# Anaesthesiaye/sound_event_detection_transformer

Measured on AMD Instinct MI355X. Metric: audio clips/sec training throughput (B=64, 10s@64-mel), higher is better.
Workload: dtype bf16; 1 GPU; URBAN-SED SEDT enc_layers=3 dec_at num_queries=10 B=64/GPU, 10 s @ 64-mel (B,1,500,64), full train step: fwd + Hungarian matching (device) + SetCriterion + bwd + clip 0.1 + AdamW, dropout 0.1; global_batch=64, parallelism=dp1

## Files before the change

include/sedt_hip.h:

```cpp
#ifndef SEDT_HIP_H
#define SEDT_HIP_H
#include <stddef.h>
#include <stdint.h>

#ifdef __cplusplus
extern "C" {
#endif

#define SEDT_F32 0
#define SEDT_BF16 1
#define SEDT_BF16X3 2

#define SEDT_ACT_NONE 0
#define SEDT_ACT_RELU 1
#define SEDT_ACT_SIGMOID 2

const char* sedt_last_error(void);
int sedt_version(void);

typedef struct SedtIgemm {
  int32_t M, N, K;
  const void* A;
  const void* B;
  int64_t lda, ldb;
  int32_t trans, conv, transposed;
  int32_t Hi, Wi, Ci, Ho, Wo;
  int32_t KH, KW, sh, sw, ph, pw, dh, dw;
  void* C;
  int64_t ldc;
  int32_t out_f32;
  const float* scale;
  const float* bias;
  const void* res;
  int64_t ldr;
  int32_t res_mod;
  const void* mask;
  int64_t ldm;
  int32_t act, act_post_res;
  float alpha;
  float drop_p;
  uint32_t seed;
  const uint32_t* seed_ptr;
  int32_t splitk;
  float* slab;
  int32_t tile_m, tile_n;
  float* colsum_out;
  uint8_t* bits_out;
  int64_t ldbits;
  int32_t mask_bits;
  int32_t f32ep;
  int32_t omap;
  int32_t o_Hi, o_Wi, o_sh, o_sw, o_h0, o_w0;
  int32_t btap_on;
  int32_t btap[8];
  void* split_out;
  int32_t awrap;
  int32_t pad2_;
  const void* bfrag;
} SedtIgemm;

int sedt_igemm(const SedtIgemm* args, int dtype, void* stream);
int sedt_sizeof(int which);
int sedt_igemm_group(const SedtIgemm* jobs, int njobs, int dtype, void* stream);
int sedt_wgrad_group(const SedtIgemm* jobs, int njobs, int dtype, void* stream);
int sedt_igemm_co(const SedtIgemm* main, const SedtIgemm* wjobs, int nw, int dtype, void* stream, int* taken);
int sedt_igemm_splitk(int M, int N, int K, int dtype);
int sedt_igemm_describe(const SedtIgemm* args, int dtype, int grouped, char* out, int cap);
int sedt_igemm_group_describe(const SedtIgemm* jobs, int njobs, int dtype, char* out, int cap);

int sedt_wgrad_reduce(const float* slab, int splitk, int R, int taps, int Ci, const float* rowscale,
                      float* out, void* stream);
int sedt_wgrad_reduce_bias(const float* slab, int splitk, int R, int taps, int Ci, const float* rowscale, float* out,
                           const float* colsum_slab, float* bias_out, void* stream);

typedef struct SedtPrefetch {
  const void* ptr[3];
  size_t bytes[3];
} SedtPrefetch;

typedef struct SedtSplitJob {
  const float* src;
  int64_t ld;
  void* dst;
  int32_t rows, cols, pattern;
  int32_t blk0;
} SedtSplitJob;
int sedt_split3(const SedtSplitJob* jobs, int njobs, void* stream);

#define SEDT_MAX_REDUCE_JOBS 40
typedef struct SedtReduceJob {
  const float* slab;
  const float* rowscale;
// ... 337 lines not shown
```

sound_event_detection_transformer_amd/csrc/igemm.hip:

```cpp
#include <stdlib.h>
#include "common.h"

namespace sedt {

template <typename T> struct Cfg;
template <> struct Cfg<float> {
  static constexpr int BK = 32, PITCH = 33, EPC = 4, KSTEP = 2, UK = 1;
};
template <> struct Cfg<bf16_t> {
  static constexpr int BK = 64, PITCH = 72, EPC = 8, KSTEP = 16, UK = 4;
};

struct GatherGeom {
  int Hi, Wi, Ci, Ho, Wo, KH, KW, sh, sw, ph, pw, dh, dw, transposed;
};

__device__ __forceinline__ long gather_pix(const GatherGeom& g, int n, int ho, int wo, int kh, int kw) {
  int hi, wi;
  if (!g.transposed) {
    hi = ho * g.sh - g.ph + kh * g.dh;
    wi = wo * g.sw - g.pw + kw * g.dw;
    if ((unsigned)hi >= (unsigned)g.Hi || (unsigned)wi >= (unsigned)g.Wi) return -1;
  } else {
    int th = ho + g.ph - kh * g.dh, tw = wo + g.pw - kw * g.dw;
// ... 369 lines not shown
#pragma unroll
        for (int j = 0; j < NI; ++j) b[j] = cB[j * 32 * PITCH + kk + kofs];
#pragma unroll
        for (int i = 0; i < MI; ++i)
#pragma unroll
          for (int j = 0; j < NI; ++j)
            acc[i][j] = __builtin_amdgcn_mfma_f32_32x32x2f32(a[i], b[j], acc[i][j], 0, 0, 0);
      }
    }
  };

  if (nkb > 0) {
    load_tiles(kb_begin, ra0, rb0);
    if (nkb > 1) load_tiles(kb_begin + 1, ra1, rb1);
    store_tiles(0, ra0, rb0);
    __syncthreads();
    auto body = [&](int it, uint4(&fa)[NRA], uint4(&fb)[NRB], const uint4(&na)[NRA], const uint4(&nb)[NRB]) {
      if (it + 2 < nkb) load_tiles(kb_begin + it + 2, fa, fb);
      compute(it & 1);
      if (it + 1 < nkb) store_tiles((it & 1) ^ 1, na, nb);
      __syncthreads();
    };
    for (int it = 0; it < nkb; it += 2) {
      body(it, ra0, rb0, ra1, rb1);
      if (it + 1 < nkb) body(it + 1, ra1, rb1, ra0, rb0);
    }
  }

  const bool slab = p.splitk > 1;
  const uint32_t seed = eff_seed(p.seed, p.seed_ptr);
  const uint32_t thresh = drop_threshold(p.drop_p);
  const float inv_keep = p.drop_p > 0.f ? 1.f / (1.f - p.drop_p) : 1.f;
  const T* resT = reinterpret_cast<const T*>(p.res);
  const T* maskT = p.mask_bits ? nullptr : reinterpret_cast<const T*>(p.mask);
  const uint8_t* maskB = p.mask_bits ? reinterpret_cast<const uint8_t*>(p.mask) : nullptr;
  auto epilogue_tile = [&](const f32x16& a, const int i, const int j) {
    const int col = n0 + wn + j * 32 + (lane & 31);
    const bool colok = col < p.N;
    float sc = 1.f, bi = 0.f;
    if (!slab && colok) {
      if (p.scale) sc = p.scale[col];
      if (p.bias) bi = p.bias[col];
    }
#pragma unroll
    for (int r = 0; r < 16; ++r) {
      const int row = m0 + wm + i * 32 + (r & 3) + 8 * (r >> 2) + 4 * (lane >> 5);
      if (p.bits_out && !slab) {
        const bool ok = row < p.M && colok;
        float v = 0.f;
        if (ok) {
          v = a[r] * sc + bi;
          if (!p.act_post_res) {
            if (p.act == SEDT_ACT_RELU) v = fmaxf(v, 0.f);
            else if (p.act == SEDT_ACT_SIGMOID) v = 1.f / (1.f + __expf(-v));
          }
          if (p.drop_p > 0.f) v = drop_keep(seed, (uint64_t)row * (uint64_t)p.N + col, thresh) ? v * inv_keep : 0.f;
          if (resT) {
            long rr = p.res_mod > 0 ? (row % p.res_mod) : row;
            v += (float)resT[rr * p.ldr + col];
          }
          if (p.act_post_res) {
            if (p.act == SEDT_ACT_RELU) v = fmaxf(v, 0.f);
            else if (p.act == SEDT_ACT_SIGMOID) v = 1.f / (1.f + __expf(-v));
          }
          if (maskT) v = ((float)maskT[(long)row * p.ldm + col] > 0.f) ? v : 0.f;
          if (maskB) v = ((maskB[(long)row * p.ldm + (col >> 3)] >> (col & 7)) & 1) ? v : 0.f;
          v *= p.alpha;
          if (p.out_f32) reinterpret_cast<float*>(p.C)[(long)row * p.ldc + col] = v;
          else { const T tv = (T)v; reinterpret_cast<T*>(p.C)[(long)row * p.ldc + col] = tv; v = (float)tv; }
        }
        const unsigned long long pos = __ballot(ok && v > 0.f);
        if (ok && (lane & 7) == 0) p.bits_out[(long)row * p.ldbits + (col >> 3)] = (uint8_t)(pos >> (lane & ~7));
        continue;
      }
      if (!(row < p.M && colok)) continue;
      float v = a[r];
      if (slab) {
        p.slab[((long)blockIdx.z * p.M + row) * p.N + col] = v;
        continue;
      }
      v = v * sc + bi;
      if (!p.act_post_res) {
        if (p.act == SEDT_ACT_RELU) v = fmaxf(v, 0.f);
        else if (p.act == SEDT_ACT_SIGMOID) v = 1.f / (1.f + __expf(-v));
      }
      if (p.drop_p > 0.f) v = drop_keep(seed, (uint64_t)row * (uint64_t)p.N + col, thresh) ? v * inv_keep : 0.f;
      if (resT) {
        long rr = p.res_mod > 0 ? (row % p.res_mod) : row;
        v += (float)resT[rr * p.ldr + col];
      }
      if (p.act_post_res) {
        if (p.act == SEDT_ACT_RELU) v = fmaxf(v, 0.f);
        else if (p.act == SEDT_ACT_SIGMOID) v = 1.f / (1.f + __expf(-v));
      }
      if (maskT) v = ((float)maskT[(long)row * p.ldm + col] > 0.f) ? v : 0.f;
      if (maskB) v = ((maskB[(long)row * p.ldm + (col >> 3)] >> (col & 7)) & 1) ? v : 0.f;
      v *= p.alpha;
      if (p.out_f32) reinterpret_cast<float*>(p.C)[(long)row * p.ldc + col] = v;
      else reinterpret_cast<T*>(p.C)[(long)row * p.ldc + col] = (T)v;
    }
  };
  epilogue_tile(acc[0][0], 0, 0);
  if constexpr (NI > 1) epilogue_tile(acc[0][1], 0, 1);
  if constexpr (MI > 1) epilogue_tile(acc[1][0], 1, 0);
  if constexpr (MI > 1 && NI > 1) epilogue_tile(acc[1][1], 1, 1);
}

template <typename T, int BM, int BN, bool TRANS, bool X3 = false, bool FAST = false>
static int launch_cfg(const SedtIgemm& p, int vecA, int vecB, hipStream_t st) {
  if constexpr (!FAST && sizeof(T) == 4) {
    if (vecA && vecB && p.M % BM == 0 && p.N % BN == 0 && p.K % (X3 ? X3BK : Cfg<T>::BK) == 0 && (!p.conv || p.trans || p.Ci % (X3 ? X3BK : Cfg<T>::BK) == 0))
      return launch_cfg<T, BM, BN, TRANS, X3, true>(p, vecA, vecB, st);
  }
  SEDT_DESCRIBE("igemm_kernel<%s, %d, %d, %s%s%s>", sizeof(T) == 4 ? "float" : "__bf16", BM, BN, TRANS ? "true" : "false", X3 ? ", true" : "",
                FAST ? (X3 ? ", true" : ", false, true") : "");
  constexpr size_t lds = X3 ? (size_t)(BM + BN) * X3P * sizeof(bf16_t) * 2 * 2 : (size_t)(BM + BN) * Cfg<T>::PITCH * sizeof(T) * 2;
  static bool attr_set = false;
  auto kern = igemm_kernel<T, BM, BN, TRANS, X3, FAST>;
  if (!attr_set) {
    hipError_t e = hipFuncSetAttribute(reinterpret_cast<const void*>(kern), hipFuncAttributeMaxDynamicSharedMemorySize,
                                       (int)lds);
    if (e != hipSuccess) {
// ... 20 lines not shown
    if (!p.trans) SEDT_REQUIRE(p.Ci % (X3 ? X3BK : Cfg<T>::BK) == 0, "igemm: conv needs Ci %% BK == 0 (Ci=%d, BK=%d)", p.Ci, X3 ? X3BK : Cfg<T>::BK);
  }
  if (!p.trans) {
    if (p.K % EPC != 0) { vecA = 0; vecB = 0; }
  }
  int bm = p.tile_m, bn = p.tile_n;
  if (bm == 0 || bn == 0) {
    bm = 64; bn = 64;
    static int gen_tile = [] { const char* e = dev_getenv("SEDT_GEN_TILE"); return e ? atoi(e) : 0; }();
    static int gen_min = [] { const char* e = dev_getenv("SEDT_GEN_TILE_MIN"); return e ? atoi(e) : 512; }();
    if (gen_tile && sizeof(T) == 4) {
      const int tm = gen_tile / 1000 >= 128 ? 128 : 64, tn = gen_tile % 1000 >= 128 ? 128 : 64;
      if (p.M % tm == 0 && p.N % tn == 0 && (long)(p.M / tm) * (p.N / tn) * (p.splitk > 1 ? p.splitk : 1) >= gen_min) { bm = tm; bn = tn; }
    }
  }
  if (p.splitk > 1) SEDT_REQUIRE(p.slab != nullptr, "igemm: splitk > 1 needs a slab");
#define SEDT_DISPATCH(BM_, BN_)                                                         \
  if (bm == BM_ && bn == BN_) {                                                         \
    return p.trans ? launch_cfg<T, BM_, BN_, true, X3>(p, vecA, vecB, st)               \
                   : launch_cfg<T, BM_, BN_, false, X3>(p, vecA, vecB, st);             \
  }
  SEDT_DISPATCH(128, 128)
  SEDT_DISPATCH(128, 64)
  SEDT_DISPATCH(64, 64)
#undef SEDT_DISPATCH
  set_error("igemm: unsupported tile %dx%d", bm, bn);
  return 1;
}

}

namespace sedt { int igemm_lds_try(const SedtIgemm& p, hipStream_t st); }

static bool use_lds_family() {
  static int v = -1;
  if (v < 0) {
    const char* e = sedt::dev_getenv("SEDT_IGEMM_LDS");
    v = (e && e[0] == '0') ? 0 : 1;
  }
  return v == 1;
}

extern "C" int sedt_igemm(const SedtIgemm* args, int dtype, void* stream) {
  using namespace sedt;
  SEDT_REQUIRE(args != nullptr, "igemm: null args");
  SEDT_REQUIRE(args->M > 0 && args->N > 0 && args->K > 0, "igemm: bad dims M=%d N=%d K=%d", args->M, args->N, args->K);
  SEDT_REQUIRE(args->A && args->B && (args->C || args->splitk > 1), "igemm: null operand");
  hipStream_t st = reinterpret_cast<hipStream_t>(stream);
  if (dtype != SEDT_BF16)
    SEDT_REQUIRE(!args->omap && !args->btap_on && !args->f32ep && !args->awrap, "igemm: omap / btap / f32ep / awrap are features of the bf16 LDS-DMA kernels");
  if (dtype == SEDT_F32) {
    SEDT_REQUIRE(args->colsum_out == nullptr, "igemm: colsum_out is a bf16-only feature");
    return launch_typed<float>(*args, st);
  }
  if (dtype == SEDT_BF16X3) {
    SEDT_REQUIRE(args->colsum_out == nullptr, "igemm: colsum_out is a bf16-only feature");
    return launch_typed<float, true>(*args, st);
  }
  if (dtype == SEDT_BF16) {
    if (use_lds_family()) {
      int r = igemm_lds_try(*args, st);
      if (r >= 0) return r;
    }
    SEDT_REQUIRE(args->colsum_out == nullptr, "igemm: colsum_out needs the bf16 LDS-DMA wgrad kernel (M,N,lda,ldb %% 8 == 0)");
    SEDT_REQUIRE(!args->omap && !args->btap_on && !args->f32ep && !args->awrap,
                 "igemm: omap / btap / f32ep / awrap problem outside the LDS-DMA envelope (M %d N %d K %d)", args->M, args->N, args->K);
    return launch_typed<bf16_t>(*args, st);
  }
  set_error("igemm: unsupported dtype %d", dtype);
  return 1;
}

namespace sedt {
thread_local Describe describe = {false, {0}};
bool wgrad4_ok(const SedtIgemm& p);
int wgrad_lds_envelope(const SedtIgemm& p, long* a_bytes, long* b_bytes);
}

extern "C" int sedt_igemm_describe(const SedtIgemm* args, int dtype, int grouped, char* out, int cap) {
  using namespace sedt;
  SEDT_REQUIRE(args && out && cap > 0, "igemm_describe: bad arguments");
  out[0] = 0;
  if (grouped && dtype == SEDT_BF16 && args->trans) {
    long a, b;
    if (wgrad_lds_envelope(*args, &a, &b) == 0) {
      snprintf(out, cap, "%s", wgrad4_ok(*args) ? "wgrad4_group_kernel" : "wgrad3_group_kernel");
      return 0;
    }
  }
  describe.on = true;
  describe.name[0] = 0;
  const int r = sedt_igemm(args, dtype, nullptr);
  describe.on = false;
  if (r == 0) snprintf(out, cap, "%s", describe.name);
  return r;
}

namespace sedt {
int wgrad3_group_try(const SedtIgemm* jobs, int njobs, hipStream_t st);
bool wgrad4_shape_ok(int M, int N);
int wgrad4_tile_m(int M, int N);
int igemm3_group_try(const SedtIgemm* jobs, int njobs, hipStream_t st);
}

extern "C" int sedt_igemm_group(const SedtIgemm* jobs, int njobs, int dtype, void* stream) {
  SEDT_REQUIRE(jobs && njobs >= 1, "igemm_group: bad arguments");
  if (dtype == SEDT_BF16 && njobs >= 2) {
    const int r = sedt::igemm3_group_try(jobs, njobs, reinterpret_cast<hipStream_t>(stream));
    if (r >= 0) return r;
  }
  for (int i = 0; i < njobs; ++i)
    if (int r = sedt_igemm(&jobs[i], dtype, stream)) return r;
  return 0;
}

extern "C" int sedt_igemm_group_describe(const SedtIgemm* jobs, int njobs, int dtype, char* out, int cap) {
  using namespace sedt;
  SEDT_REQUIRE(jobs && njobs >= 1 && out && cap > 0, "igemm_group_describe: bad arguments");
  out[0] = 0;
  if (dtype != SEDT_BF16 || njobs < 2) return 0;
  describe.on = true;
  describe.name[0] = 0;
  const int r = igemm3_group_try(jobs, njobs, nullptr);
  describe.on = false;
  if (r == 0) snprintf(out, cap, "%s", describe.name);
  return r > 0 ? r : 0;
}

extern "C" int sedt_wgrad_group(const SedtIgemm* jobs, int njobs, int dtype, void* stream) {
  SEDT_REQUIRE(jobs && njobs >= 1, "wgrad_group: bad arguments");
  if (dtype == SEDT_BF16) {
    const int r = sedt::wgrad3_group_try(jobs, njobs, reinterpret_cast<hipStream_t>(stream));
    if (r >= 0) return r;
  }
  for (int i = 0; i < njobs; ++i)
    if (int r = sedt_igemm(&jobs[i], dtype, stream)) return r;
  return 0;
}

#include "wgrad3_body.h"
namespace sedt {
int wgrad3_group_build(const SedtIgemm* jobs, int njobs, WgradGroup* g);
extern thread_local const WgradGroup* co_group;
extern thread_local bool co_taken;
}

extern "C" int sedt_igemm_co(const SedtIgemm* main, const SedtIgemm* wjobs, int nw, int dtype, void* stream, int* taken) {
  using namespace sedt;
  SEDT_REQUIRE(main && (nw == 0 || wjobs) && taken, "igemm_co: bad arguments");
  *taken = 0;
  if (nw == 0) return sedt_igemm(main, dtype, stream);
  static int on = -1;
  if (on < 0) {
    const char* e = sedt::dev_getenv("SEDT_COSCHEDULE");
    on = (e && e[0] == '0') ? 0 : 1;
  }
  WgradGroup g;
  bool grouped = on && dtype == SEDT_BF16 && main->trans == 0 && wgrad3_group_build(wjobs, nw, &g) == 0;
  co_taken = false;
  co_group = grouped ? &g : nullptr;
  const int r = sedt_igemm(main, dtype, stream);
  co_group = nullptr;
  *taken = co_taken ? 1 : 0;
  return r;
}

extern "C" int sedt_igemm_splitk(int M, int N, int K, int dtype) {
  static int target_env = -2;
  if (target_env == -2) {
    const char* e = sedt::dev_getenv("SEDT_SPLITK_TARGET");
    target_env = e ? atoi(e) : -1;
  }
  const int target = target_env > 0 ? target_env : (dtype == SEDT_BF16 ? 384 : 768);
  int bk = dtype == SEDT_BF16 ? 64 : 32;
  long tiles = (long)((M + 63) / 64) * ((N + 63) / 64);
  int nkb = (K + bk - 1) / bk;
  int tgt = target;
  if (dtype == SEDT_BF16 && sedt::wgrad4_shape_ok(M, N)) {
    static int wide_env = -2;
    if (wide_env == -2) {
      const char* e = sedt::dev_getenv("SEDT_SPLITK_TARGET_WIDE");
      wide_env = e ? atoi(e) : -1;
    }
// ... 28 lines not shown
```

sound_event_detection_transformer_amd/csrc/igemm3.hip:

```cpp
#include <stdlib.h>
#include <type_traits>
#include "wgrad3_body.h"

namespace sedt {

__device__ __forceinline__ int uniform_i32(int v) { return __builtin_amdgcn_readfirstlane(v); }
typedef __attribute__((ext_vector_type(4))) unsigned u32x4;

__device__ __attribute__((used)) unsigned char g_code_tail_pad[64 * 1024];

#ifdef SEDT_DEV
__device__ unsigned long long g_phase_ts[5 * 4096];
__device__ int g_ts_filter[3];
#define SEDT_TS_INIT() \
  const bool ts_on_ = threadIdx.x == 0 && bx < 4096 && (g_ts_filter[0] == 0 || (g_ts_filter[0] == p.M && g_ts_filter[1] == p.N && g_ts_filter[2] == p.K))
#define SEDT_TS(i_, v_)                              \
  do {                                               \
    if (ts_on_) g_phase_ts[bx * 5 + (i_)] = (v_);    \
  } while (0)
#else
#define SEDT_TS_INIT() do {} while (0)
#define SEDT_TS(i_, v_) do {} while (0)
#endif

template <int BM, int BN, int S, int NW, bool CONV, int PP = 0, int KH = 1, int BR = 0>
__device__ __forceinline__ void igemm3_impl(const SedtIgemm& p, const unsigned a_bytes_flag, const unsigned b_bytes_flag, const int bx) {
  const unsigned b_bytes = b_bytes_flag & 0x7fffffffu;
  const unsigned a_bytes = a_bytes_flag & 0x7fffffffu;
  constexpr int WM = BR ? BM : BM / 2, WN = BR ? BN / 4 : BN / 2, MI = WM / 32, NI = WN / 32;
  constexpr int STAGE_BYTES = (BM + (BR ? 0 : BN)) * ROWB;
  constexpr int GA = BM / (8 * NW), GB = BR ? 0 : BN / (8 * NW);
  constexpr int NT = NW * KH * 64;
  static_assert(NW == 4 || NW == 8, "4 or 8 waves");
  static_assert(KH == 1 || (KH == 2 && NW == 8 && PP), "two K halves: the ping-pong 8-wave form only");
  static_assert(GA >= 1 && (BR || GB >= 1), "tile too small for the wave count");
  static_assert(!BR || (NW == 8 && PP && KH == 1 && BN == 128), "register-streamed B: the 8-wave ping-pong form, 128 columns");
  constexpr unsigned OOB = 0x80000000u;
  extern __shared__ __attribute__((aligned(16))) unsigned char smem[];
  SEDT_TS_INIT();
  SEDT_TS(0, __builtin_amdgcn_s_memtime());
  SEDT_TS(4, __builtin_amdgcn_s_memrealtime());

  const int t = threadIdx.x, lane = t & 63;
  const int wave_all = uniform_i32(t >> 6);
  const int khalf = KH == 2 ? wave_all >> 3 : 0;
  const int wave = KH == 2 ? (wave_all & 7) : wave_all;
  const int kgrp = wave >> 2;
  const int wm = BR ? 0 : ((wave & 3) >> 1) * WM, wn = BR ? (wave & 3) * WN : (wave & 1) * WN;
  unsigned char* const ring = smem + khalf * (S * STAGE_BYTES);

  const int ntn = (p.N + BN - 1) / BN, ntm = (p.M + BM - 1) / BM;
  const int nwg = ntn * ntm;
  int vid;
  {
    const int b = bx, xcd = b & 7, q = nwg >> 3, r = nwg & 7;
    vid = (xcd < r ? xcd * (q + 1) : r * (q + 1) + (xcd - r) * q) + (b >> 3);
// ... 19 lines not shown
      const unsigned total = BR ? (unsigned)((long)p.N * p.ldb * 2) : b_bytes;
      const unsigned chunk = ((total + npf - 1) / npf + 127u) & ~127u;
      const unsigned lo = (unsigned)bx * chunk, hi = lo + chunk < total ? lo + chunk : total;
#pragma unroll
      for (int i = 0; i < 4; ++i) {
        const unsigned off = lo + (unsigned)i * 8192u + (unsigned)lane * 128u;
        if (lo + (unsigned)i * 8192u < hi)
          __builtin_amdgcn_raw_ptr_buffer_load_lds(BR ? rsF0 : rsB, (lds_void*)(ring), 4, off < hi ? off : OOB, 0, 0, 0);
      }
    }
  }

  constexpr int CPR = BN / 8;
  constexpr int NCH = (BM * CPR + NT - 1) / NT;
  constexpr bool PARTIAL = BM * CPR % NT != 0;
  static_assert(!PARTIAL || NCH == 1, "epilogue chunks must divide evenly, or be fewer than the threads");
  const bool f32ep = p.f32ep != 0;
  const bf16_t* resT = f32ep ? nullptr : reinterpret_cast<const bf16_t*>(p.res);
  const bool mbits = p.mask_bits != 0;
  const bf16_t* maskT = (mbits || f32ep) ? nullptr : reinterpret_cast<const bf16_t*>(p.mask);
  const float* resF = f32ep ? reinterpret_cast<const float*>(p.res) : nullptr;
  const float* maskF = (f32ep && !mbits) ? reinterpret_cast<const float*>(p.mask) : nullptr;
  const uint8_t* maskB = mbits ? reinterpret_cast<const uint8_t*>(p.mask) : nullptr;
  constexpr bool LATE = BM > 128;
  bf16x8 res_pf[LATE ? 1 : NCH], mask_pf[LATE ? 1 : NCH];
  uint32_t mbit_pf[LATE ? 1 : NCH];
  auto out_row = [&](const int row) -> long {
    if (!p.omap) return row;
    const int hw = p.Ho * p.Wo;
    const int n = row / hw, rem = row - n * hw;
    const int ho = rem / p.Wo, wo = rem - ho * p.Wo;
    return ((long)n * p.o_Hi + ho * p.o_sh + p.o_h0) * p.o_Wi + wo * p.o_sw + p.o_w0;
  };
  if constexpr (!LATE) {
#pragma unroll
  for (int c = 0; c < NCH; ++c) {
    const int u = t + c * NT;
    const int row = m0 + u / CPR, col = n0 + (u % CPR) * 8;
    if (row < p.M && col < p.N && (!PARTIAL || u < BM * CPR)) {
      const long orow = out_row(row);
      if (resT) {
        long rrow = orow;
        if (p.res_mod > 0) rrow = orow % p.res_mod;
        res_pf[c] = *reinterpret_cast<const bf16x8*>(resT + rrow * p.ldr + col);
      }
      if (maskT) mask_pf[c] = *reinterpret_cast<const bf16x8*>(maskT + orow * p.ldm + col);
      if (maskB) mbit_pf[c] = maskB[orow * p.ldm + (col >> 3)];
    }
  }
  }

  static_assert(NT % CPR == 0, "column of a thread's chunks must not depend on the chunk");
  constexpr bool EARLY_AFFINE = NW == 8 && !LATE;
  const int ccol = n0 + (t % CPR) * 8;
  const bool col_ok = ccol < p.N;
  float sc8[8], bi8[8];
  auto load_affine = [&]() {
#pragma unroll
    for (int e = 0; e < 8; ++e) { sc8[e] = 1.f; bi8[e] = 0.f; }
    if (col_ok && p.scale) {
      const float4 s0 = *reinterpret_cast<const float4*>(p.scale + ccol), s1 = *reinterpret_cast<const float4*>(p.scale + ccol + 4);
      sc8[0] = s0.x; sc8[1] = s0.y; sc8[2] = s0.z; sc8[3] = s0.w; sc8[4] = s1.x; sc8[5] = s1.y; sc8[6] = s1.z; sc8[7] = s1.w;
    }
    if (col_ok && p.bias) {
      const float4 s0 = *reinterpret_cast<const float4*>(p.bias + ccol), s1 = *reinterpret_cast<const float4*>(p.bias + ccol + 4);
      bi8[0] = s0.x; bi8[1] = s0.y; bi8[2] = s0.z; bi8[3] = s0.w; bi8[4] = s1.x; bi8[5] = s1.y; bi8[6] = s1.z; bi8[7] = s1.w;
    }
  };
  if constexpr (EARLY_AFFINE) load_affine();

  const int lrow = lane >> 3, pc = lane & 7;
  const int taps = CONV ? p.KH * p.KW : 1;
  const int sg = (CONV && p.transposed) ? -1 : 1;
  const long tsub = (CONV && p.transposed) ? p.lda / p.sh : p.lda;
  unsigned a_off[GA], a_mask[GA];
#pragma unroll
  for (int i = 0; i < GA; ++i) {
// ... 291 lines not shown
    {
      const float4 x0 = *reinterpret_cast<const float4*>(Cs + trow * CP + cc);
      const float4 x1 = *reinterpret_cast<const float4*>(Cs + trow * CP + cc + 4);
      v[0] = x0.x; v[1] = x0.y; v[2] = x0.z; v[3] = x0.w; v[4] = x1.x; v[5] = x1.y; v[6] = x1.z; v[7] = x1.w;
      if (TWO_CS) {
#pragma unroll
        for (int gq = 1; gq < 2 * KH; ++gq) {
          const float4 y0 = *reinterpret_cast<const float4*>(Cs2 + (gq - 1) * (BM * CP) + trow * CP + cc);
          const float4 y1 = *reinterpret_cast<const float4*>(Cs2 + (gq - 1) * (BM * CP) + trow * CP + cc + 4);
          v[0] += y0.x; v[1] += y0.y; v[2] += y0.z; v[3] += y0.w; v[4] += y1.x; v[5] += y1.y; v[6] += y1.z; v[7] += y1.w;
        }
      }
    }
    if (affine) {
#pragma unroll
      for (int e = 0; e < 8; ++e) v[e] = fmaf(v[e], sc8[e], bi8[e]);
    }
    if (relu_pre) {
#pragma unroll
      for (int e = 0; e < 8; ++e) v[e] = fmaxf(v[e], 0.f);
    }
    if (p.drop_p > 0.f) {
      const uint64_t h0 = ((uint64_t)orow * (uint64_t)p.N + col) >> 1;
      const uint32_t lo = (uint32_t)h0;
      const uint32_t inner = mix32(seed ^ ((uint32_t)(h0 >> 32) * 0x9E3779B9U) ^ 0x85ebca6bU);
#pragma unroll
      for (int q = 0; q < 4; ++q) {
        const uint32_t h = mix32((lo + q) ^ inner);
        v[2 * q] = (h & 0xffffu) >= thresh ? v[2 * q] * inv_keep : 0.f;
        v[2 * q + 1] = (h >> 16) >= thresh ? v[2 * q + 1] * inv_keep : 0.f;
      }
    }
    if (resT) {
      bf16x8 rv;
      if constexpr (LATE) {
        long rrow = orow;
        if (p.res_mod > 0) rrow = orow % p.res_mod;
        rv = *reinterpret_cast<const bf16x8*>(resT + rrow * p.ldr + col);
      } else {
        rv = res_pf[c];
      }
#pragma unroll
      for (int e = 0; e < 8; ++e) v[e] += (float)rv[e];
    }
    if (resF) {
      long rrow = orow;
      if (p.res_mod > 0) rrow = orow % p.res_mod;
      const float4 r0 = *reinterpret_cast<const float4*>(resF + rrow * p.ldr + col);
      const float4 r1 = *reinterpret_cast<const float4*>(resF + rrow * p.ldr + col + 4);
      v[0] += r0.x; v[1] += r0.y; v[2] += r0.z; v[3] += r0.w; v[4] += r1.x; v[5] += r1.y; v[6] += r1.z; v[7] += r1.w;
    }
    if (relu_post) {
#pragma unroll
      for (int e = 0; e < 8; ++e) v[e] = fmaxf(v[e], 0.f);
    }
    if (maskT) {
      bf16x8 mv;
      if constexpr (LATE) mv = *reinterpret_cast<const bf16x8*>(maskT + orow * p.ldm + col);
      else mv = mask_pf[c];
#pragma unroll
      for (int e = 0; e < 8; ++e) v[e] = ((float)mv[e] > 0.f) ? v[e] : 0.f;
    }
    if (maskF) {
      const float4 q0 = *reinterpret_cast<const float4*>(maskF + orow * p.ldm + col);
      const float4 q1 = *reinterpret_cast<const float4*>(maskF + orow * p.ldm + col + 4);
      const float mv[8] = {q0.x, q0.y, q0.z, q0.w, q1.x, q1.y, q1.z, q1.w};
#pragma unroll
      for (int e = 0; e < 8; ++e) v[e] = mv[e] > 0.f ? v[e] : 0.f;
    }
    if (maskB) {
      uint32_t mb;
      if constexpr (LATE) mb = maskB[orow * p.ldm + (col >> 3)];
      else mb = mbit_pf[c];
#pragma unroll
      for (int e = 0; e < 8; ++e) v[e] = ((mb >> e) & 1u) ? v[e] : 0.f;
    }
    if (p.alpha != 1.f) {
#pragma unroll
      for (int e = 0; e < 8; ++e) v[e] *= p.alpha;
    }
    if (f32ep) {
      float* outF = reinterpret_cast<float*>(p.C) + orow * p.ldc + col;
      *reinterpret_cast<float4*>(outF) = make_float4(v[0], v[1], v[2], v[3]);
// ... 536 lines not shown
```

sound_event_detection_transformer_amd/functional.py:

```python
import torch
from torch.autograd import Function

from . import ops, packing, runtime
from .lib import F32, BF16
from .ops import ACT_NONE, ACT_RELU, ACT_SIGMOID, ConvGeom


def _dt_of(t):
    return F32 if t.dtype == torch.float32 else BF16


def _as(t, dt):
    want = torch.float32 if dt == F32 else torch.bfloat16
    t = t.contiguous()
    return t if t.dtype == want else ops.cast(t, dt)


def _wf(dt, w):
    return w if dt == F32 else ops.cast(w, BF16)


def _wb(dt, w):
    return ops.pack_conv(dt, w, want_fwd=False)[1]

# ... 858 lines not shown
                _, _, ga = ops.bneck_bwd(gp, B, r['H'], r['W'], r['chain'], *r['ab_bits'], None, chain_only=True)
                side = ops.conv_dgrad(dt, gp, B, r['gd'], r['wdb'])
                mask_x = (not first) or meta['mask_input']
                ep = (dict(mask=r['x'], ldm=r['x'].stride(0)) if mask_x else {})
                gp = ops.conv_dgrad(dt, ga, B, r['g1'], w1b, res=side, ldr=side.stride(0), **ep)
                continue
            if r.get('fused') is not None and want_gx:
                mask_x = (not first) or meta['mask_input']
                if not mask_x or r.get('xbits') is not None:
                    train_w = t[0].requires_grad or t[5].requires_grad or t[10].requires_grad
                    prev = saved[bi_ - 1] if bi_ > 0 else None
                    nx = prev['fused'] if (prev is not None and prev.get('fused') is not None and blk.cin == 1024) else None
                    gx, gb, ga = ops.bneck_bwd(gp, B, r['H'], r['W'], r['fused'], *r['ab_bits'], r['xbits'] if mask_x else None, want_g=train_w,
                                               nxt=nx)
                    if t[10].requires_grad:
                        grads[base + 10] = ops.wgrad(dt, gp, r['b'], B, r['g3'], rowscale=s3, batch=rb, param=t[10])
                    if t[5].requires_grad:
                        grads[base + 5] = ops.wgrad(dt, gb, r['a'], B, r['g2'], rowscale=s2, batch=rb, param=t[5])
                    if t[0].requires_grad:
                        grads[base + 0] = ops.wgrad(dt, ga, r['x'], B, r['g1'], rowscale=s1, batch=rb, param=t[0])
                    gp = gx
                    continue
            if t[10].requires_grad:
                grads[base + 10] = ops.wgrad(dt, gp, r['b'], B, r['g3'], rowscale=s3, batch=rb, param=t[10])
            gb = ops.conv_dgrad(dt, gp, B, r['g3'], w3b, mask=r['b'], ldm=r['b'].stride(0))
            if t[5].requires_grad:
                grads[base + 5] = ops.wgrad(dt, gb, r['a'], B, r['g2'], rowscale=s2, batch=rb, param=t[5])
            ga = ops.conv_dgrad(dt, gb, B, r['g2'], w2b, mask=r['a'], ldm=r['a'].stride(0))
            if t[0].requires_grad:
                grads[base + 0] = ops.wgrad(dt, ga, r['x'], B, r['g1'], rowscale=s1, batch=rb, param=t[0])
            if blk.ds and t[15].requires_grad:
                grads[base + 15] = ops.wgrad(dt, gp, r['x'], B, r['gd'], rowscale=r['sd'], batch=rb, param=t[15])
            if want_gx:
                side = ops.conv_dgrad(dt, gp, B, r['gd'], r['wdb']) if blk.ds else gp
                mask_x = (not first) or meta['mask_input']
                if mask_x and r.get('xbits') is not None:
                    ep = dict(mask=r['xbits'], ldm=r['xbits'].stride(0), mask_bits=True)
                else:
                    ep = dict(mask=r['x'], ldm=r['x'].stride(0)) if mask_x else {}
                gp = ops.conv_dgrad(dt, ga, B, r['g1'], w1b, res=side, ldr=side.stride(0), **ep)
            else:
                gp = None
        rb.flush(prefetch=ctx.bwd_next)
        ctx.saved = None
        return (gp, None) + tuple(grads)
```

sound_event_detection_transformer_amd/lib.py:

```python
import ctypes as C
import os

import torch

HERE = os.path.dirname(os.path.abspath(__file__))
LIB_PATH = os.path.join(HERE, 'libsedt_hip.so')
if os.environ.get('SEDT_LIB_AB') and os.environ.get('SEDT_DEV') == '1':
    LIB_PATH = os.environ['SEDT_LIB_AB']

F32, BF16 = 0, 1
BF16X3 = 2
GEMM_X3 = False


def gemm_dtype(dtype):
    return BF16X3 if (dtype == F32 and GEMM_X3) else dtype
ACT_NONE, ACT_RELU, ACT_SIGMOID = 0, 1, 2
TORCH_DTYPE = {F32: torch.float32, BF16: torch.bfloat16}


class SedtIgemm(C.Structure):
    _fields_ = [
        ('M', C.c_int32), ('N', C.c_int32), ('K', C.c_int32),
        ('A', C.c_void_p), ('B', C.c_void_p),
        ('lda', C.c_int64), ('ldb', C.c_int64),
        ('trans', C.c_int32), ('conv', C.c_int32), ('transposed', C.c_int32),
        ('Hi', C.c_int32), ('Wi', C.c_int32), ('Ci', C.c_int32), ('Ho', C.c_int32), ('Wo', C.c_int32),
        ('KH', C.c_int32), ('KW', C.c_int32), ('sh', C.c_int32), ('sw', C.c_int32), ('ph', C.c_int32),
        ('pw', C.c_int32), ('dh', C.c_int32), ('dw', C.c_int32),
        ('C', C.c_void_p), ('ldc', C.c_int64), ('out_f32', C.c_int32),
        ('scale', C.c_void_p), ('bias', C.c_void_p),
        ('res', C.c_void_p), ('ldr', C.c_int64), ('res_mod', C.c_int32),
        ('mask', C.c_void_p), ('ldm', C.c_int64),
        ('act', C.c_int32), ('act_post_res', C.c_int32),
        ('alpha', C.c_float), ('drop_p', C.c_float), ('seed', C.c_uint32), ('seed_ptr', C.c_void_p),
        ('splitk', C.c_int32), ('slab', C.c_void_p),
        ('tile_m', C.c_int32), ('tile_n', C.c_int32),
        ('colsum_out', C.c_void_p),
        ('bits_out', C.c_void_p), ('ldbits', C.c_int64), ('mask_bits', C.c_int32), ('f32ep', C.c_int32),
        ('omap', C.c_int32), ('o_Hi', C.c_int32), ('o_Wi', C.c_int32), ('o_sh', C.c_int32), ('o_sw', C.c_int32), ('o_h0', C.c_int32),
        ('o_w0', C.c_int32), ('btap_on', C.c_int32), ('btap', C.c_int32 * 8), ('split_out', C.c_void_p), ('awrap', C.c_int32), ('pad2_', C.c_int32), ('bfrag', C.c_void_p),
    ]


class SedtReduceJob(C.Structure):
    _fields_ = [('slab', C.c_void_p), ('rowscale', C.c_void_p), ('out', C.c_void_p), ('colsum_slab', C.c_void_p),
                ('bias_out', C.c_void_p), ('splitk', C.c_int32), ('R', C.c_int32), ('taps', C.c_int32), ('Ci', C.c_int32),
                ('blk0', C.c_int32), ('cs_splitk', C.c_int32)]


CRIT_MAXL = 8


class SedtCriterion(C.Structure):
    _fields_ = [(n, C.c_void_p) for n in ('logits', 'boxes', 'at', 'tc', 'coef', 'wbox', 'tbox', 'gt_weak', 'tgt_len',
                                           'num_boxes', 'empty_weight', 'dlogits', 'dboxes', 'dboxes2', 'dat', 'out')] + \
               [(n, C.c_int32) for n in ('L', 'B', 'ns', 'Q', 'C', 'n_lab', 'Bat')] + \
               [('layer_of', C.c_int32 * CRIT_MAXL), ('w_ce', C.c_float * CRIT_MAXL), ('w_bbox', C.c_float * CRIT_MAXL),
                ('w_giou', C.c_float * CRIT_MAXL), ('w_weak', C.c_float), ('fl', C.c_int32), ('alpha_fl', C.c_float),
                ('gamma_fl', C.c_float), ('nonfinite', C.c_void_p), ('split', C.c_void_p), ('Qs', C.c_int32), ('q0', C.c_int32),
                ('total', C.c_void_p), ('at_p', C.c_void_p), ('dat_p', C.c_void_p), ('w_weak_p', C.c_float), ('wp_all', C.c_int32),
                ('Bp', C.c_int32)]


class SedtPoolAt(C.Structure):
    _fields_ = [('logits', C.c_void_p), ('boxes', C.c_void_p), ('attn', C.c_void_p)] + \
               [(n, C.c_int32) for n in ('B', 'Qs', 'q0', 'Q', 'C', 'mode')]


POOL_MODES = {'max': 0, 'avg': 1, 'attn': 2, 'weighted_sum': 3}


class SedtMatch(C.Structure):
    _fields_ = [(n, C.c_void_p) for n in ('logits', 'boxes', 'lab_cat', 'lab_off', 'box_cat', 'box_off', 'ratio_cat', 'tc',
# ... 191 lines not shown
```

sound_event_detection_transformer_amd/ops.py:

```python
import ctypes as C

import os
import numpy as np
import torch

from . import lib as L
from .lib import F32, BF16, ACT_NONE, ACT_RELU, ACT_SIGMOID, TORCH_DTYPE, p as _p


class ConvGeom(object):
    __slots__ = ('Hi', 'Wi', 'Ci', 'Ho', 'Wo', 'Co', 'KH', 'KW', 'sh', 'sw', 'ph', 'pw', 'dh', 'dw')

    def __init__(self, Hi, Wi, Ci, Co, k=1, stride=1, pad=0, dil=1):
        self.Hi, self.Wi, self.Ci, self.Co = Hi, Wi, Ci, Co
        self.KH = self.KW = k
        self.sh = self.sw = stride
        self.ph = self.pw = pad
        self.dh = self.dw = dil
        self.Ho = (Hi + 2 * pad - dil * (k - 1) - 1) // stride + 1
        self.Wo = (Wi + 2 * pad - dil * (k - 1) - 1) // stride + 1

    @property
    def taps(self):
        return self.KH * self.KW

    @property
    def plain(self):
        return self.KH == 1 and self.KW == 1 and self.sh == 1 and self.sw == 1 and self.ph == 0 and self.pw == 0


def _dev_env(name, default):
    return os.environ.get(name, default) if os.environ.get('SEDT_DEV') == '1' else default


IGEMM_BREG = _dev_env('SEDT_IGEMM_BREG', '0') != '0'
RELU_BITS = _dev_env('SEDT_RELU_BITS', '1') != '0'
PROFILE = None
PROFILE_FUSED = []
PROFILE_HINT = None


def _dev_check(*ts):
    for t in ts:
        if t is not None and not t.is_cuda:
            raise RuntimeError('sedt ops need GPU tensors: the HIP path has no CPU fallback')


def igemm_args(M, N, K, A, lda, B, ldb, Cout, ldc, *, trans=0, conv=None, transposed=0, out_f32=0, scale=None,
               bias=None, res=None, ldr=0, res_mod=0, mask=None, ldm=0, act=ACT_NONE, act_post_res=0, alpha=1.0, drop_p=0.0,
               seed=0, seed_ptr=None, splitk=1, slab=None, tile=(0, 0), colsum_out=None, mask_bits=False, bits_out=None):
    _dev_check(A, B, Cout)
    a = L.SedtIgemm()
    a.M, a.N, a.K = M, N, K
    a.A, a.B, a.lda, a.ldb = A.data_ptr(), B.data_ptr(), lda, ldb
    a.trans, a.transposed = trans, transposed
    if conv is not None:
        a.conv = 1
        (a.Hi, a.Wi, a.Ci, a.Ho, a.Wo, a.KH, a.KW, a.sh, a.sw, a.ph, a.pw, a.dh, a.dw) = conv
    else:
        a.conv = 0
        a.KH = a.KW = a.sh = a.sw = a.dh = a.dw = 1
    a.C = Cout.data_ptr() if Cout is not None else None
    a.ldc, a.out_f32 = ldc, out_f32
    a.scale = scale.data_ptr() if scale is not None else None
    a.bias = bias.data_ptr() if bias is not None else None
    a.res = res.data_ptr() if res is not None else None
    a.ldr, a.res_mod = ldr, res_mod
    a.mask = mask.data_ptr() if mask is not None else None
    a.ldm = ldm
    a.act, a.act_post_res, a.alpha = act, act_post_res, alpha
    a.drop_p, a.seed = drop_p, seed & 0xffffffff
    a.seed_ptr = seed_ptr.data_ptr() if seed_ptr is not None else None
    a.splitk = splitk
    a.slab = slab.data_ptr() if slab is not None else None
    a.tile_m, a.tile_n = tile
    a.colsum_out = colsum_out.data_ptr() if colsum_out is not None else None
    if mask_bits:
        assert mask is not None and mask.dtype == torch.uint8
        a.mask_bits = 1
    if bits_out is not None:
        assert bits_out.dtype == torch.uint8 and bits_out.shape == (M, N // 8) and N % 8 == 0 and bits_out.stride(1) == 1 and not trans
        a.bits_out, a.ldbits = bits_out.data_ptr(), bits_out.stride(0)
    if IGEMM_BREG and not trans and B.dtype == torch.bfloat16:
        from . import packing
        fr = packing.lookup_operand_frag(B.data_ptr())
        if fr is not None and fr.numel() == B.numel() and ldb * B.shape[0] == B.numel():
            a.bfrag = fr.data_ptr()
    return a


class WgradPool(object):
    SLOTS = 1280
    MAX_RIDERS = 10

    def __init__(self):
        self.gemms, self.reduces, self.keep, self.dtype = [], [], [], None

    def push(self, group, dtype, jobs, keep, operands):
        self.gemms.extend(group)
        self.reduces.extend(jobs)
# ... 433 lines not shown
        t, w = _split3([(t, 0, B * g.Hi * g.Wi, cin, t.stride(0), 0), (w, 0, cout * 9, cin, cin, 1)])
        w = w.view(cout, 27 * cin)
        C = 3 * cin
    jobs = []
    for half in (0, 1):
        kw0 = (1 - half) if not transposed else half
        conv = (g.Hi, g.Wi, C, g.Ho, d, 3, 2, 1, 1, d, (d if transposed else 0), d, d)
        a = igemm_args(B * g.Ho * d, cout, 6 * C, t, t.stride(0), w, w.stride(0), out, out.stride(0), conv=conv, transposed=int(transposed),
                       tile=(128, 128), out_f32=int(x3), **ep)
        a.omap, a.o_Hi, a.o_Wi, a.o_sh, a.o_sw, a.o_h0, a.o_w0 = 1, g.Ho, g.Wo, 1, 1, 0, half * d
        a.btap_on, a.f32ep, a.awrap = 1, int(x3), (cin if x3 else 0)
        for kh in range(3):
            for j in range(2):
                a.btap[kh * 2 + j] = (kh * 3 + kw0 + j) * C
        jobs.append(a)
    if describe:
        return _group_label(jobs)
    arr = (L.SedtIgemm * 2)(*jobs)
    L.check(L.load().sedt_igemm_group(arr, 2, BF16, L.stream_ptr()), 'igemm_group_dil')
    return out


def conv_dgrad(dtype, dy, B, g, wb, out=None, **ep):
    M = B * g.Hi * g.Wi
    if out is None:
        out = torch.empty((M, g.Ci), device=dy.device, dtype=TORCH_DTYPE[dtype])
    if _dgrad_s2_ok(dtype, dy, g, wb, out, ep):
        return _conv_dgrad_s2(dy, B, g, wb, out, ep, x3=dtype == F32)
    if _dil_halves_ok(dtype, dy, g, wb, out, ep, True):
        return _conv_dil_halves(dy, B, g, wb, out, ep, True, dtype == F32)
    if _conv3_c64_ok(dtype, dy, g, ep, out) and 'scale' not in ep and 'bias' not in ep:
        return _conv3_c64(dy, B, g, wb, 1, out, ep)
    conv = None if g.plain else _geom_tuple(g, transposed=True)
    global PROFILE_HINT
    if PROFILE is not None and _conv3_c64_ok(dtype, dy, g, ep, out, True) and 'scale' not in ep and 'bias' not in ep:
        PROFILE_HINT = 'conv3x3_c64_kernel'
    elif PROFILE is not None and dtype == BF16 and _dgrad_s2_ok(dtype, dy, g, wb, out, ep, True):
        PROFILE_HINT = ('group', _conv_dgrad_s2(dy, B, g, wb, out, ep, describe=True), 0.25)
    elif PROFILE is not None and dtype == BF16 and _dil_halves_ok(dtype, dy, g, wb, out, ep, True, True):
        PROFILE_HINT = ('group', _conv_dil_halves(dy, B, g, wb, out, ep, True, False, describe=True), 2.0 / 3.0)
    igemm(dtype, M, g.Ci, g.taps * g.Co, dy, dy.stride(0), wb, g.taps * g.Co, out, out.stride(0), conv=conv,
          transposed=0 if g.plain else 1, **ep)
    PROFILE_HINT = None
    return out


def _fused_bias_ok(dtype, dy, x, g):
    return (dtype == BF16 and L.load() is not None and g.Co % 8 == 0 and (g.taps * g.Ci) % 8 == 0 and dy.stride(0) % 8 == 0
            and x.stride(0) % 8 == 0 and dy.data_ptr() % 16 == 0 and x.data_ptr() % 16 == 0 and g.Ci % 8 == 0)


class ReduceBatch(object):

    def __init__(self, shared=False):
        self.jobs, self.keep, self.deferred, self.operands = [], [], [], []
        self.group, self.group_dtype = [], None
        self.shared = shared
        self.expect = []

    def add_gemm(self, dtype, args, shape, code=None):
        self.group.append((args, shape, L.gemm_dtype(dtype) if code is None else code))
        self.group_dtype = dtype

    def _launch_group(self):
        if not self.group:
            return
        lib = L.load()
        if PROFILE is not None:
            for a, shape, code in self.group:
                L.check(lib.sedt_igemm(C.byref(a), code, L.stream_ptr()), 'sedt_igemm')
                PROFILE.append((a, code, shape, (list(self.keep), list(self.operands)), 'wgrad_group'))
        else:
            i = 0
            while i < len(self.group):
                j = i
                while j < len(self.group) and self.group[j][2] == self.group[i][2]:
                    j += 1
# ... 1032 lines not shown
```

Measured before the change: 12640 clips/s.

## Compute strided 1x1 projection dgrad compactly and scatter via residual row map

For downsampling residual blocks with a strided 1x1 projection, the input gradient of the projection is now computed as a plain GEMM over only the Ho*Wo output positions instead of a transposed-gather conv over the full Hi*Wi grid, which is mostly zeros. The compact result is fed as the residual to the main conv dgrad, and a new packed rmap field lets the epilogue map each full-resolution row to its compact row, adding nothing where the stride skips it. This removes redundant FLOPs and a full-size intermediate, at the cost of integer div/mod work per epilogue row and an extra branch in the residual path of every kernel.

Result: faster. 12840 clips/s, median of 6 (+1.6%).

```diff
diff --git a/include/sedt_hip.h b/include/sedt_hip.h
--- a/include/sedt_hip.h
+++ b/include/sedt_hip.h
@@ -55,9 +55,10 @@
   int32_t btap[8];
   void* split_out;
   int32_t awrap;
-  int32_t pad2_;
+  int32_t rmap;
   const void* bfrag;
 } SedtIgemm;
+#define SEDT_RMAP(r_Hi, r_Wi, r_sh, r_sw) ((int32_t)((uint32_t)(r_Hi) | (uint32_t)(r_Wi) << 12 | (uint32_t)(r_sh) << 24 | (uint32_t)(r_sw) << 28))
 
 int sedt_igemm(const SedtIgemm* args, int dtype, void* stream);
 int sedt_sizeof(int which);
diff --git a/sound_event_detection_transformer_amd/csrc/igemm.hip b/sound_event_detection_transformer_amd/csrc/igemm.hip
--- a/sound_event_detection_transformer_amd/csrc/igemm.hip
+++ b/sound_event_detection_transformer_amd/csrc/igemm.hip
@@ -425,6 +425,19 @@
   const uint32_t thresh = drop_threshold(p.drop_p);
   const float inv_keep = p.drop_p > 0.f ? 1.f / (1.f - p.drop_p) : 1.f;
   const T* resT = reinterpret_cast<const T*>(p.res);
+  auto res_row = [&](const int row, long& rr) -> bool {
+    rr = row;
+    if (p.res_mod > 0) {
+      rr = row % p.res_mod;
+    } else if (p.rmap) {
+      const unsigned rm = (unsigned)p.rmap;
+      const int rHi = rm & 0xfffu, rWi = (rm >> 12) & 0xfffu, rsh = (rm >> 24) & 15u, rsw = rm >> 28;
+      const int n = row / (rHi * rWi), rem = row - n * (rHi * rWi), h = rem / rWi, w = rem - h * rWi;
+      if (h % rsh != 0 || w % rsw != 0) return false;
+      rr = ((long)n * ((rHi - 1) / rsh + 1) + h / rsh) * ((rWi - 1) / rsw + 1) + w / rsw;
+    }
+    return true;
+  };
   const T* maskT = p.mask_bits ? nullptr : reinterpret_cast<const T*>(p.mask);
   const uint8_t* maskB = p.mask_bits ? reinterpret_cast<const uint8_t*>(p.mask) : nullptr;
   auto epilogue_tile = [&](const f32x16& a, const int i, const int j) {
@@ -449,8 +462,8 @@
           }
           if (p.drop_p > 0.f) v = drop_keep(seed, (uint64_t)row * (uint64_t)p.N + col, thresh) ? v * inv_keep : 0.f;
           if (resT) {
-            long rr = p.res_mod > 0 ? (row % p.res_mod) : row;
-            v += (float)resT[rr * p.ldr + col];
+            long rr;
+            if (res_row(row, rr)) v += (float)resT[rr * p.ldr + col];
           }
           if (p.act_post_res) {
             if (p.act == SEDT_ACT_RELU) v = fmaxf(v, 0.f);
@@ -479,8 +492,8 @@
       }
       if (p.drop_p > 0.f) v = drop_keep(seed, (uint64_t)row * (uint64_t)p.N + col, thresh) ? v * inv_keep : 0.f;
       if (resT) {
-        long rr = p.res_mod > 0 ? (row % p.res_mod) : row;
-        v += (float)resT[rr * p.ldr + col];
+        long rr;
+        if (res_row(row, rr)) v += (float)resT[rr * p.ldr + col];
       }
       if (p.act_post_res) {
         if (p.act == SEDT_ACT_RELU) v = fmaxf(v, 0.f);
@@ -567,6 +580,25 @@
 
 namespace sedt { int igemm_lds_try(const SedtIgemm& p, hipStream_t st); }
 
+static int check_rmap(const SedtIgemm& p) {
+  if (!p.rmap) return 0;
+  const unsigned rm = (unsigned)p.rmap;
+  const long rHi = rm & 0xfffu, rWi = (rm >> 12) & 0xfffu, rsh = (rm >> 24) & 15u, rsw = rm >> 28;
+  SEDT_REQUIRE(p.res != nullptr && p.res_mod == 0 && !p.trans && p.splitk <= 1,
+               "igemm: rmap needs a residual, res_mod == 0, trans == 0 and no split-K (res %p res_mod %d trans %d splitk %d)", p.res, p.res_mod,
+               p.trans, p.splitk);
+  SEDT_REQUIRE(rHi >= 1 && rWi >= 1 && rsh >= 1 && rsw >= 1, "igemm: rmap %ld x %ld / (%ld, %ld): every part must be >= 1", rHi, rWi, rsh, rsw);
+  long pixels = p.M;
+  if (p.omap) {
+    SEDT_REQUIRE(p.conv && p.Ho > 0 && p.Wo > 0 && p.M % (p.Ho * p.Wo) == 0 && p.o_Hi == rHi && p.o_Wi == rWi,
+                 "igemm: rmap %ld x %ld over an omap image of %d x %d", rHi, rWi, p.o_Hi, p.o_Wi);
+    pixels = (long)(p.M / (p.Ho * p.Wo)) * p.o_Hi * p.o_Wi;
+  }
+  SEDT_REQUIRE(pixels % (rHi * rWi) == 0 && pixels < (1L << 24),
+               "igemm: rmap %ld x %ld needs a whole number of images and fewer than 2^24 output pixels (%ld)", rHi, rWi, pixels);
+  return 0;
+}
+
 static bool use_lds_family() {
   static int v = -1;
   if (v < 0) {
@@ -582,6 +614,7 @@
   SEDT_REQUIRE(args->M > 0 && args->N > 0 && args->K > 0, "igemm: bad dims M=%d N=%d K=%d", args->M, args->N, args->K);
   SEDT_REQUIRE(args->A && args->B && (args->C || args->splitk > 1), "igemm: null operand");
   hipStream_t st = reinterpret_cast<hipStream_t>(stream);
+  if (int r = check_rmap(*args)) return r;
   if (dtype != SEDT_BF16)
     SEDT_REQUIRE(!args->omap && !args->btap_on && !args->f32ep && !args->awrap, "igemm: omap / btap / f32ep / awrap are features of the bf16 LDS-DMA kernels");
   if (dtype == SEDT_F32) {
@@ -640,6 +673,8 @@
 
 extern "C" int sedt_igemm_group(const SedtIgemm* jobs, int njobs, int dtype, void* stream) {
   SEDT_REQUIRE(jobs && njobs >= 1, "igemm_group: bad arguments");
+  for (int i = 0; i < njobs; ++i)
+    if (int r = check_rmap(jobs[i])) return r;
   if (dtype == SEDT_BF16 && njobs >= 2) {
     const int r = sedt::igemm3_group_try(jobs, njobs, reinterpret_cast<hipStream_t>(stream));
     if (r >= 0) return r;
@@ -664,6 +699,7 @@
 
 extern "C" int sedt_wgrad_group(const SedtIgemm* jobs, int njobs, int dtype, void* stream) {
   SEDT_REQUIRE(jobs && njobs >= 1, "wgrad_group: bad arguments");
+  for (int i = 0; i < njobs; ++i) SEDT_REQUIRE(!jobs[i].rmap, "wgrad_group: a weight-gradient problem takes no residual map (job %d)", i);
   if (dtype == SEDT_BF16) {
     const int r = sedt::wgrad3_group_try(jobs, njobs, reinterpret_cast<hipStream_t>(stream));
     if (r >= 0) return r;
@@ -684,6 +720,7 @@
   using namespace sedt;
   SEDT_REQUIRE(main && (nw == 0 || wjobs) && taken, "igemm_co: bad arguments");
   *taken = 0;
+  for (int i = 0; i < nw; ++i) SEDT_REQUIRE(!wjobs[i].rmap, "igemm_co: a weight-gradient rider takes no residual map (job %d)", i);
   if (nw == 0) return sedt_igemm(main, dtype, stream);
   static int on = -1;
   if (on < 0) {
diff --git a/sound_event_detection_transformer_amd/csrc/igemm3.hip b/sound_event_detection_transformer_amd/csrc/igemm3.hip
--- a/sound_event_detection_transformer_amd/csrc/igemm3.hip
+++ b/sound_event_detection_transformer_amd/csrc/igemm3.hip
@@ -22,6 +22,29 @@
 #define SEDT_TS_INIT() do {} while (0)
 #define SEDT_TS(i_, v_) do {} while (0)
 #endif
+
+__device__ __noinline__ long rmap_row(const int orow, const unsigned rm) {
+  const int rHi = rm & 0xfffu, rWi = (rm >> 12) & 0xfffu, rsh = (rm >> 24) & 15u, rsw = rm >> 28;
+  auto divmod = [](const int a, const int b, int& q, int& r) {
+    q = (int)((float)a * (1.f / (float)b));
+    r = a - q * b;
+    if (r < 0) { --q; r += b; }
+    if (r >= b) { ++q; r -= b; }
+  };
+  int n, rem, h, w;
+  divmod(orow, rHi * rWi, n, rem);
+  divmod(rem, rWi, h, w);
+  if (((rsh & (rsh - 1)) | (rsw & (rsw - 1))) == 0) {
+    const int lh = __builtin_ctz(rsh), lw = __builtin_ctz(rsw);
+    if (((h & (rsh - 1)) | (w & (rsw - 1))) != 0) return -1;
+    return ((long)n * (((rHi - 1) >> lh) + 1) + (h >> lh)) * (((rWi - 1) >> lw) + 1) + (w >> lw);
+  }
+  int hc, hr, wc, wr;
+  divmod(h, rsh, hc, hr);
+  divmod(w, rsw, wc, wr);
+  if (hr != 0 || wr != 0) return -1;
+  return ((long)n * ((rHi - 1) / rsh + 1) + hc) * ((rWi - 1) / rsw + 1) + wc;
+}
 
 template <int BM, int BN, int S, int NW, bool CONV, int PP = 0, int KH = 1, int BR = 0>
 __device__ __forceinline__ void igemm3_impl(const SedtIgemm& p, const unsigned a_bytes_flag, const unsigned b_bytes_flag, const int bx) {
@@ -107,6 +130,17 @@
     const int ho = rem / p.Wo, wo = rem - ho * p.Wo;
     return ((long)n * p.o_Hi + ho * p.o_sh + p.o_h0) * p.o_Wi + wo * p.o_sw + p.o_w0;
   };
+  const uint4 NEG_ZERO8 = make_uint4(0x80008000u, 0x80008000u, 0x80008000u, 0x80008000u);
+  auto res_row = [&](const long orow, long& rrow) -> bool {
+    rrow = orow;
+    if (p.res_mod > 0) {
+      rrow = orow % p.res_mod;
+    } else if (p.rmap) {
+      rrow = rmap_row((int)orow, (unsigned)p.rmap);
+      if (rrow < 0) return false;
+    }
+    return true;
+  };
   if constexpr (!LATE) {
 #pragma unroll
   for (int c = 0; c < NCH; ++c) {
@@ -115,9 +149,9 @@
     if (row < p.M && col < p.N && (!PARTIAL || u < BM * CPR)) {
       const long orow = out_row(row);
       if (resT) {
-        long rrow = orow;
-        if (p.res_mod > 0) rrow = orow % p.res_mod;
-        res_pf[c] = *reinterpret_cast<const bf16x8*>(resT + rrow * p.ldr + col);
+        long rrow;
+        if (res_row(orow, rrow)) res_pf[c] = *reinterpret_cast<const bf16x8*>(resT + rrow * p.ldr + col);
+        else res_pf[c] = __builtin_bit_cast(bf16x8, NEG_ZERO8);
       }
       if (maskT) mask_pf[c] = *reinterpret_cast<const bf16x8*>(maskT + orow * p.ldm + col);
       if (maskB) mbit_pf[c] = maskB[orow * p.ldm + (col >> 3)];
@@ -475,23 +509,25 @@
       }
     }
     if (resT) {
-      bf16x8 rv;
       if constexpr (LATE) {
-        long rrow = orow;
-        if (p.res_mod > 0) rrow = orow % p.res_mod;
-        rv = *reinterpret_cast<const bf16x8*>(resT + rrow * p.ldr + col);
+        long rrow;
+        if (res_row(orow, rrow)) {
+          const bf16x8 rv = *reinterpret_cast<const bf16x8*>(resT + rrow * p.ldr + col);
+#pragma unroll
+          for (int e = 0; e < 8; ++e) v[e] += (float)rv[e];
+        }
       } else {
-        rv = res_pf[c];
-      }
-#pragma unroll
-      for (int e = 0; e < 8; ++e) v[e] += (float)rv[e];
+#pragma unroll
+        for (int e = 0; e < 8; ++e) v[e] += (float)res_pf[c][e];
+      }
     }
     if (resF) {
-      long rrow = orow;
-      if (p.res_mod > 0) rrow = orow % p.res_mod;
-      const float4 r0 = *reinterpret_cast<const float4*>(resF + rrow * p.ldr + col);
-      const float4 r1 = *reinterpret_cast<const float4*>(resF + rrow * p.ldr + col + 4);
-      v[0] += r0.x; v[1] += r0.y; v[2] += r0.z; v[3] += r0.w; v[4] += r1.x; v[5] += r1.y; v[6] += r1.z; v[7] += r1.w;
+      long rrow;
+      if (res_row(orow, rrow)) {
+        const float4 r0 = *reinterpret_cast<const float4*>(resF + rrow * p.ldr + col);
+        const float4 r1 = *reinterpret_cast<const float4*>(resF + rrow * p.ldr + col + 4);
+        v[0] += r0.x; v[1] += r0.y; v[2] += r0.z; v[3] += r0.w; v[4] += r1.x; v[5] += r1.y; v[6] += r1.z; v[7] += r1.w;
+      }
     }
     if (relu_post) {
 #pragma unroll
diff --git a/sound_event_detection_transformer_amd/functional.py b/sound_event_detection_transformer_amd/functional.py
--- a/sound_event_detection_transformer_amd/functional.py
+++ b/sound_event_detection_transformer_amd/functional.py
@@ -914,13 +914,13 @@
             if blk.ds and t[15].requires_grad:
                 grads[base + 15] = ops.wgrad(dt, gp, r['x'], B, r['gd'], rowscale=r['sd'], batch=rb, param=t[15])
             if want_gx:
-                side = ops.conv_dgrad(dt, gp, B, r['gd'], r['wdb']) if blk.ds else gp
+                side, ep_side = ops.proj_dgrad(dt, gp, B, r['gd'], r['wdb']) if blk.ds else (gp, dict(ldr=gp.stride(0)))
                 mask_x = (not first) or meta['mask_input']
                 if mask_x and r.get('xbits') is not None:
                     ep = dict(mask=r['xbits'], ldm=r['xbits'].stride(0), mask_bits=True)
                 else:
                     ep = dict(mask=r['x'], ldm=r['x'].stride(0)) if mask_x else {}
-                gp = ops.conv_dgrad(dt, ga, B, r['g1'], w1b, res=side, ldr=side.stride(0), **ep)
+                gp = ops.conv_dgrad(dt, ga, B, r['g1'], w1b, res=side, **ep_side, **ep)
             else:
                 gp = None
         rb.flush(prefetch=ctx.bwd_next)
diff --git a/sound_event_detection_transformer_amd/lib.py b/sound_event_detection_transformer_amd/lib.py
--- a/sound_event_detection_transformer_amd/lib.py
+++ b/sound_event_detection_transformer_amd/lib.py
@@ -39,7 +39,7 @@
         ('colsum_out', C.c_void_p),
         ('bits_out', C.c_void_p), ('ldbits', C.c_int64), ('mask_bits', C.c_int32), ('f32ep', C.c_int32),
         ('omap', C.c_int32), ('o_Hi', C.c_int32), ('o_Wi', C.c_int32), ('o_sh', C.c_int32), ('o_sw', C.c_int32), ('o_h0', C.c_int32),
-        ('o_w0', C.c_int32), ('btap_on', C.c_int32), ('btap', C.c_int32 * 8), ('split_out', C.c_void_p), ('awrap', C.c_int32), ('pad2_', C.c_int32), ('bfrag', C.c_void_p),
+        ('o_w0', C.c_int32), ('btap_on', C.c_int32), ('btap', C.c_int32 * 8), ('split_out', C.c_void_p), ('awrap', C.c_int32), ('rmap', C.c_int32), ('bfrag', C.c_void_p),
     ]
 
 
diff --git a/sound_event_detection_transformer_amd/ops.py b/sound_event_detection_transformer_amd/ops.py
--- a/sound_event_detection_transformer_amd/ops.py
+++ b/sound_event_detection_transformer_amd/ops.py
@@ -48,7 +48,7 @@
 
 def igemm_args(M, N, K, A, lda, B, ldb, Cout, ldc, *, trans=0, conv=None, transposed=0, out_f32=0, scale=None,
                bias=None, res=None, ldr=0, res_mod=0, mask=None, ldm=0, act=ACT_NONE, act_post_res=0, alpha=1.0, drop_p=0.0,
-               seed=0, seed_ptr=None, splitk=1, slab=None, tile=(0, 0), colsum_out=None, mask_bits=False, bits_out=None):
+               seed=0, seed_ptr=None, splitk=1, slab=None, tile=(0, 0), colsum_out=None, mask_bits=False, bits_out=None, res_map=None):
     _dev_check(A, B, Cout)
     a = L.SedtIgemm()
     a.M, a.N, a.K = M, N, K
@@ -66,6 +66,10 @@
     a.bias = bias.data_ptr() if bias is not None else None
     a.res = res.data_ptr() if res is not None else None
     a.ldr, a.res_mod = ldr, res_mod
+    if res_map is not None:
+        r_Hi, r_Wi, r_sh, r_sw = res_map
+        assert res is not None and not res_mod and 1 <= r_Hi < 4096 and 1 <= r_Wi < 4096 and 1 <= r_sh < 16 and 1 <= r_sw < 16, res_map
+        a.rmap = C.c_int32(r_Hi | r_Wi << 12 | r_sh << 24 | r_sw << 28).value
     a.mask = mask.data_ptr() if mask is not None else None
     a.ldm = ldm
     a.act, a.act_post_res, a.alpha = act, act_post_res, alpha
@@ -565,6 +569,8 @@
     if _conv3_c64_ok(dtype, dy, g, ep, out) and 'scale' not in ep and 'bias' not in ep:
         return _conv3_c64(dy, B, g, wb, 1, out, ep)
     conv = None if g.plain else _geom_tuple(g, transposed=True)
+    if L.LAUNCH_LOG is not None and not g.plain:
+        L.LAUNCH_LOG['conv_dgrad_gather:k%ds%d' % (g.KH, g.sh)] += 1
     global PROFILE_HINT
     if PROFILE is not None and _conv3_c64_ok(dtype, dy, g, ep, out, True) and 'scale' not in ep and 'bias' not in ep:
         PROFILE_HINT = 'conv3x3_c64_kernel'
@@ -576,6 +582,25 @@
           transposed=0 if g.plain else 1, **ep)
     PROFILE_HINT = None
     return out
+
+
+PROJ_COMPACT = _dev_env('SEDT_PROJ_COMPACT', '1') != '0'
+
+
+def proj_compact_ok(g):
+    return PROJ_COMPACT and g.KH == 1 and g.KW == 1 and (g.sh > 1 or g.sw > 1) and g.ph == 0 and g.pw == 0 and g.dh == 1 and g.dw == 1
+
+
+def proj_dgrad(dtype, dy, B, g, wb):
+    if not proj_compact_ok(g):
+        side = conv_dgrad(dtype, dy, B, g, wb)
+        return side, dict(ldr=side.stride(0))
+    M = B * g.Ho * g.Wo
+    side = torch.empty((M, g.Ci), device=dy.device, dtype=TORCH_DTYPE[dtype])
+    if L.LAUNCH_LOG is not None:
+        L.LAUNCH_LOG['proj_dgrad:%dx%dx%d' % (M, g.Ci, g.Co)] += 1
+    igemm(dtype, M, g.Ci, g.Co, dy, dy.stride(0), wb, g.Co, side, side.stride(0))
+    return side, dict(ldr=side.stride(0), res_map=(g.Hi, g.Wi, g.sh, g.sw))
 
 
 def _fused_bias_ok(dtype, dy, x, g):
```
